# ModelTC/llmc

Hardware: AMD Instinct MI355X
Metric: layers/sec (GPTQ W4A16, Llama-3-8B Linear shapes, 128x2048 calib) (higher is better)
Workload: dtype bf16

## Files before the change

include/llmc_hip.h:

```cpp
#ifndef LLMC_HIP_H_
#define LLMC_HIP_H_

#include <stddef.h>
#include <stdint.h>

#ifdef __cplusplus
extern "C" {
#endif

#define LLMC_HIP_ABI_VERSION 1

#define LLMC_OK 0
#define LLMC_EINVAL (-22)
#define LLMC_ENOTSUP (-95)
#define LLMC_EIO (-5)

#define LLMC_F16 0
#define LLMC_BF16 1
#define LLMC_F32 2
#define LLMC_F64 3
#define LLMC_SCALAR_QPARAM 16
#define LLMC_FRACTIONAL_ZP 32

#define LLMC_OUT_FAKE 0
// ... 108 lines not shown
                                              llmc_stream_t stream);
int llmc_hessian_accum_barrier_timeouts(const void* ws, const int64_t* T_list_host, int n, int64_t K, int64_t ldx,
                                        unsigned* out_host, llmc_stream_t stream);

size_t llmc_hessian_prep_ws_bytes(int64_t K);
int llmc_hessian_prep(float* H, const void* W, int wdt, int64_t R, int64_t K, const int64_t* perm,
                      float percdamp, float* Hout, float* Wout, void* ws, llmc_stream_t stream);

int llmc_gather_cols(const float* in, int64_t R, int64_t K, const int64_t* idx, float* out, llmc_stream_t stream);

size_t llmc_chol_inv_upper_ws_bytes(int64_t K);
int llmc_chol_inv_upper(float* A, int64_t K, void* ws, int32_t* info_dev, llmc_stream_t stream);
int llmc_hessian_prep_rev(float* H, const void* W, int wdt, int64_t R, int64_t K, const int64_t* perm,
                          float percdamp, float* Hout, float* Wout, void* ws, llmc_stream_t stream);
int llmc_chol_inv_upper_rev(float* Arev, float* Uout, int64_t K, void* ws, int32_t* info_dev, llmc_stream_t stream);

size_t llmc_gptq_quantize_ws_bytes(int64_t R, int64_t K);
int llmc_gptq_quantize(float* W, const float* Hinv, int64_t R, int64_t K, int sym, float qmin,
                       float qmax, int64_t group_size, int static_groups, const int32_t* col_group,
                       float* scales, float* zeros, float* Wout, float* losses, int blocksize,
                       void* ws, llmc_stream_t stream);
int llmc_gptq_quantize_cols(float* W, const float* Hinv, int64_t R, int64_t K, int64_t n_quant, int sym, float qmin,
                       float qmax, int64_t group_size, int static_groups, const int32_t* col_group,
                       float* scales, float* zeros, float* Wout, float* losses, int blocksize,
                       void* ws, llmc_stream_t stream);
int llmc_gptq_quantize_fp8_cols(float* W, const float* Hinv, int64_t R, int64_t K, int64_t n_quant, int fmt,
                                int64_t group_size, int static_groups, const int32_t* col_group, float* scales,
                                float* Wout, float* losses, int blocksize, void* ws, llmc_stream_t stream);
size_t llmc_gptq_quantize_mse_ws_bytes(int64_t R, int64_t K);
int llmc_gptq_quantize_mse(float* W, const float* Hinv, int64_t R, int64_t K, int64_t n_quant, int sym, float qmin,
// ... 134 lines not shown
```

llmc_amd/_ffi.py:

```python
import ctypes as C
import os

import torch

_HERE = os.path.dirname(os.path.abspath(__file__))
LIB_PATH = os.path.join(_HERE, 'csrc', 'libllmc_hip.so')

F16, BF16, F32 = 0, 1, 2
F64 = 3
OUT_FAKE, OUT_I32, OUT_I8, OUT_U8 = 0, 1, 2, 3
SCALAR_QPARAM = 16
LINEAR_YBLOCKED = 4
FRACTIONAL_ZP = 32
KV_REQUANT, KV_NEW_FAKE = 1, 2

_DT = {torch.float16: F16, torch.bfloat16: BF16, torch.float32: F32}

_i64, _i32, _f32, _f64, _vp, _sz = C.c_int64, C.c_int, C.c_float, C.c_double, C.c_void_p, C.c_size_t

SIGNATURES = {
    'llmc_hip_abi_version': (_i32, []),
    'llmc_hip_build_id': (C.c_char_p, []),
    'llmc_hip_last_error': (_i32, [C.c_char_p, _sz]),
    'llmc_hip_set_helper_streams': (_i32, [_i32]),
# ... 28 lines not shown
    'llmc_hessian_accum_ptrs_partials': (_i32, [_vp, _vp, _i32, _i32, _i64, _i64, _vp, _vp]),
    'llmc_hessian_accum_ptrs_reduce': (_i32, [_vp, _vp, _i32, _i64, _i64, _f64, _f64, _vp, _vp]),
    'llmc_hessian_accum_barrier_timeouts': (_i32, [_vp, _vp, _i32, _i64, _i64, _vp, _vp]),
    'llmc_hessian_max_problems': (_i32, []),
    'llmc_hessian_accum_multi_ws_bytes': (_sz, [_vp, _i32]),
    'llmc_hessian_accum_multi_partials': (_i32, [_vp, _i32, _i32, _vp, _vp]),
    'llmc_hessian_accum_multi_reduce': (_i32, [_vp, _i32, _vp, _vp]),
    'llmc_hessian_accum_multi_barrier_timeouts': (_i32, [_vp, _i32, _vp, _vp, _vp]),
    'llmc_gather_cols': (_i32, [_vp, _i64, _i64, _vp, _vp, _vp]),
    'llmc_hessian_prep_ws_bytes': (_sz, [_i64]),
    'llmc_hessian_prep': (_i32, [_vp, _vp, _i32, _i64, _i64, _vp, _f32, _vp, _vp, _vp, _vp]),
    'llmc_chol_inv_upper_ws_bytes': (_sz, [_i64]),
    'llmc_chol_inv_upper': (_i32, [_vp, _i64, _vp, _vp, _vp]),
    'llmc_hessian_prep_rev': (_i32, [_vp, _vp, _i32, _i64, _i64, _vp, _f32, _vp, _vp, _vp, _vp]),
    'llmc_chol_inv_upper_rev': (_i32, [_vp, _vp, _i64, _vp, _vp, _vp]),
    'llmc_gptq_quantize_ws_bytes': (_sz, [_i64, _i64]),
    'llmc_gptq_quantize': (_i32, [_vp, _vp, _i64, _i64, _i32, _f32, _f32, _i64, _i32, _vp, _vp, _vp, _vp, _vp,
                                  _i32, _vp, _vp]),
    'llmc_gptq_quantize_cols': (_i32, [_vp, _vp, _i64, _i64, _i64, _i32, _f32, _f32, _i64, _i32, _vp, _vp, _vp, _vp, _vp,
                                       _i32, _vp, _vp]),
    'llmc_gptq_quantize_fp8_cols': (_i32, [_vp, _vp, _i64, _i64, _i64, _i32, _i64, _i32, _vp, _vp, _vp, _vp, _i32, _vp, _vp]),
    'llmc_gptq_quantize_mse_ws_bytes': (_sz, [_i64, _i64]),
    'llmc_gptq_quantize_mse': (_i32, [_vp, _vp, _i64, _i64, _i64, _i32, _f32, _f32, _i64, _i32, _i32, _i32, _f32, _vp, _vp,
                                      _vp, _vp, _i32, _vp, _vp]),
    'llmc_spqr_quantize_ws_bytes': (_sz, [_i64, _i64]),
    'llmc_spqr_quantize': (_i32, [_vp, _vp, _i64, _i64, _f32, _f32, _i64, _f32, _i32, _f32, _f32, _f32, _f32, _vp, _vp,
                                  _vp, _vp, _vp, _i32, _vp, _vp]),
    'llmc_awq_act_mean_ws_bytes': (_sz, [_i64, _i64]),
    'llmc_awq_act_mean': (_i32, [_vp, _i32, _i64, _i64, _vp, _vp, _vp]),
    'llmc_awq_weight_mean_ws_bytes': (_sz, [_i64, _i64]),
# ... 54 lines not shown
    'llmc_kv_sink_update': (_i32, [_i32, _i64, _i64, _i64, _i64, _i64, _i64, _i64, _i64, _i64, _i64, _i64, _vp, _vp, _vp, _vp, _vp,
                                   _vp, _vp, _vp, _i64, _i64, _i64, _vp]),
    'llmc_block_influence_ws_bytes': (_sz, [_i64]),
    'llmc_block_influence': (_i32, [_vp, _vp, _i32, _i64, _i64, _i64, _i64, _i32, _vp, _vp, _vp, _vp]),
    'llmc_test_sgemm': (_i32, [_vp, _vp, _vp, _i64, _i64, _i64, _i32, _i32, _i32, _i32, _i32, _i32, _i32, _i32,
                               _i32, _i32, _vp]),
    'llmc_test_sgemm_phased': (_i32, [_vp, _vp, _vp, _i64, _i64, _i64, _i32, _i32, _i32, _i32, _i32, _vp]),
    'llmc_test_gemm3': (_i32, [_vp, _vp, _vp, _i64, _i64, _i64, _i32, _i32, _i32, _i32, _i32, _i32, _i32, _i32, _vp]),
    'llmc_test_gemm3_planes': (_i32, [_vp, _vp, _vp, _i64, _i64, _i64, _i32, _i32, _i32, _i32, _i32, _vp, _vp]),
    'llmc_test_gemm3s_stamps': (_i32, [_vp]),
    'llmc_test_gptq_rider_plan': (_i32, [_i64, _i64, _i64, _i64, _i32, _vp, _i32]),
    'llmc_test_gptq_pipe_plan': (_i32, [_i64, _i64, _i64, _i64, _i32, _vp, _i32]),
    'llmc_test_chol_plan': (_i32, [_i64, _i32, _i32, _vp, _i32]),
    'llmc_test_gemm_route': (_i32, [_vp, _vp]),
    'llmc_test_linear_route': (_i32, [_vp, _vp]),
}



class HessianProblem(C.Structure):
    _fields_ = [('H', _vp), ('dstate', _vp), ('X_list_host', _vp), ('T_list_host', _vp), ('n', _i32), ('K', _i64),
                ('ldx', _i64), ('n_before', _f64), ('n_after', _f64)]


_lib = None


class LlmcHipError(RuntimeError):
    pass

# ... 172 lines not shown
```

llmc_amd/compression/quantization/gptq_ops.py:

```python
import torch

from llmc_amd import _ffi


def hessian_prep(H, W, perm, percdamp, want_h=True, h_out=None, reverse_h=False):
    _ffi.require_gpu(H, W, perm)
    L = _ffi.lib()
    K = H.shape[0]
    Hout = None
    if want_h:
        Hout = h_out if h_out is not None else torch.empty_like(H)
    Wout = None
    R = 0
    if W is not None:
        R = W.shape[0]
        W = W.contiguous()
        Wout = torch.empty((R, K), dtype=torch.float32, device=W.device)
    ws = _ffi.workspace(L.llmc_hessian_prep_ws_bytes(K), H.device)
    if perm is not None:
        perm = perm.to(torch.int64).contiguous()
    fn = L.llmc_hessian_prep_rev if reverse_h else L.llmc_hessian_prep
    _ffi.check(fn(_ffi.ptr(H), _ffi.ptr(W), _ffi.dt(W) if W is not None else 2, R, K,
                  _ffi.ptr(perm), float(percdamp), _ffi.ptr(Hout), _ffi.ptr(Wout), _ffi.ptr(ws),
                  _ffi.stream()), 'llmc_hessian_prep')
    return Hout, Wout


GATHER_MAX_K = 40960


def gather_cols(src, idx):
    _ffi.require_gpu(src, idx)
    L = _ffi.lib()
    if src.dtype != torch.float32 or src.dim() != 2:
        raise ValueError('gather_cols: src must be fp32 [R, K]')
# ... 129 lines not shown
```

llmc_amd/compression/quantization/gptq_pipeline.py:

```python
from dataclasses import dataclass

import torch

from llmc_amd import _ffi

from . import gptq_ops
from .hessian import HessianAccumulator


@dataclass
class GptqConfig:
    bit: int = 4
    symmetric: bool = False
    group_size: int = 128
    actorder: bool = True
    static_groups: bool = False
    percdamp: float = 0.01
    blocksize: int = 128
    mse: tuple = None

    def __post_init__(self):
        if isinstance(self.bit, str):
            if self.bit not in gptq_ops.FP8_FORMATS:
                raise NotImplementedError(f"GptqConfig bit={self.bit!r}: the FP8 column loop has the e4m3 and e5m2 grids")
# ... 41 lines not shown


def _prep_and_factor(H, W, perm, percdamp, h_work):
    if _ffi.HOST_OPTIONS['k3_fused_prep']:
        Hrev, Wp = gptq_ops.hessian_prep(H, W, perm, percdamp, want_h=True, h_out=h_work, reverse_h=True)
        U, info = gptq_ops.chol_inv_upper_rev(Hrev, check=False, return_info=True)
        return U, Wp, info
    Hp, Wp = gptq_ops.hessian_prep(H, W, perm, percdamp, want_h=True, h_out=h_work)
    U, info = gptq_ops.chol_inv_upper(Hp, check=False, return_info=True)
    return U, Wp, info


def quantize_stacked(W_list, H, cfg, static_qparams=None, h_work=None, want_losses=True, rows=None):
    _ffi.require_gpu(H, *W_list)
    K = H.shape[0]
    Wcat = torch.cat([w.reshape(w.shape[0], -1) for w in W_list], dim=0) if len(W_list) > 1 else W_list[0]
    if rows is not None:
        if static_qparams is not None:
            sc = torch.cat([s.reshape(w.shape[0], -1) for (s, _), w in zip(static_qparams, W_list)], 0)[rows[0]:rows[1]]
            zr = None
            if static_qparams[0][1] is not None:
                zr = torch.cat([z.reshape(w.shape[0], -1) for (_, z), w in zip(static_qparams, W_list)], 0)[rows[0]:rows[1]]
            static_qparams = [(sc, zr)]
        W_list = [Wcat[rows[0]:rows[1]]]
        Wcat = W_list[0]
    rows = [w.shape[0] for w in W_list]
    perm = None
    if cfg.actorder:
        perm = torch.argsort(torch.diagonal(H), descending=True)
    U, Wp, info = _prep_and_factor(H, Wcat, perm, cfg.percdamp, h_work)
    qmin, qmax = cfg.qrange
    static_mode = cfg.static_groups or not cfg.group_size
# ... 72 lines not shown
```

llmc_amd/csrc/abi.hip:

```cpp
#include <mutex>
#include <set>
#include <utility>
#include "common.h"

namespace llmc {
static thread_local char g_last_error[512] = "";
static thread_local int g_helper_streams = 1;
bool helper_streams_enabled() { return g_helper_streams != 0; }
static thread_local int g_cu_reserve = 0;
int cu_reserve() { return g_cu_reserve; }
static thread_local int g_opt[OPT_COUNT] = {};
int opt(int id) { return (id >= 0 && id < OPT_COUNT) ? g_opt[id] : 0; }
static const char* const g_opt_names[OPT_COUNT] = {
    "k3_fp32", "k3_no_gemm6", "k3_no_planes", "k3_split_far", "k4_split_far", "k4_err_rowmajor", "gptq_generic",
    "gemm3_nospec", "gemm3s_min_tiles", "no_shortk", "linear_nosplit", "fp8_exact_div", "side_cu_mask", "k1_batch_off", "k1_fp32_diag", "fp8_no_packed16", "gemm3s_no_dma", "sgemm_no_wide", "gemm3_no_wide", "no_riders", "kv_sink_max_grid",
    "block_influence_max_grid"};

void set_last_error(const char* where, hipError_t e) {
    snprintf(g_last_error, sizeof(g_last_error), "%s: %s (%d)", where, hipGetErrorString(e), (int)e);
}
void set_last_error_msg(const char* msg) { snprintf(g_last_error, sizeof(g_last_error), "%s", msg); }

static std::mutex g_dev_mu;
static int g_cu_count[LLMC_MAX_DEVICES] = {};
static std::set<std::pair<int, const void*>> g_lds_attr_done;

int device_cu_count() {
    int dev = 0;
    if (hipGetDevice(&dev) != hipSuccess || dev < 0 || dev >= LLMC_MAX_DEVICES) return 256;
    std::lock_guard<std::mutex> lk(g_dev_mu);
    if (g_cu_count[dev] == 0) {
// ... 71 lines not shown
```

llmc_amd/csrc/cholesky.hip:

```cpp
#include <stdlib.h>
#include "common.h"
#include "mfma_common.h"
#include "sgemm.h"
#include "pipe_lanes.h"

namespace llmc {

static constexpr int NB = 128;

__global__ __launch_bounds__(256) void k_antitranspose(const float* __restrict__ in, float* __restrict__ out,
                                                       int n, int upper_only) {
    __shared__ float tile[32][33];
    const int tx = threadIdx.x & 31, ty = threadIdx.x >> 5;
    const int r0 = blockIdx.y * 32, c0 = blockIdx.x * 32;
    for (int y = ty; y < 32; y += 8) {
        int r = r0 + y, c = c0 + tx;
        tile[y][tx] = (r < n && c < n) ? in[(int64_t)r * n + c] : 0.0f;
    }
    __syncthreads();
    for (int y = ty; y < 32; y += 8) {
        int c = c0 + y, r = r0 + tx;
        if (r < n && c < n) {
            int orow = n - 1 - c, ocol = n - 1 - r;
            float v = tile[tx][y];
            if (upper_only && ocol < orow) v = 0.0f;
            out[(int64_t)orow * n + ocol] = v;
        }
    }
}

static constexpr int PLD = 132;

__device__ __forceinline__ float rdlane(float v, int l) {
    return __int_as_float(__builtin_amdgcn_readlane(__float_as_int(v), l));
}

__device__ __forceinline__ void wave_potrf32_inv(float* __restrict__ S, float* __restrict__ V,
                                                 float* __restrict__ rowbuf, int lane, int kglobal,
                                                 int* __restrict__ info) {
#pragma clang fp contract(fast)
    (void)rowbuf;
    const int j = lane & 31, h = lane >> 5;
    f32x16 A, E;
// ... 316 lines not shown
template <> __device__ __forceinline__ float4 load4_f32<f16_t>(const f16_t* p) {
    const uint2 u = *reinterpret_cast<const uint2*>(p);
    f16_t h[4];
    __builtin_memcpy(h, &u, 8);
    return make_float4(to_f32<f16_t>(h[0]), to_f32<f16_t>(h[1]), to_f32<f16_t>(h[2]), to_f32<f16_t>(h[3]));
}
template <> __device__ __forceinline__ float4 load4_f32<bf16_t>(const bf16_t* p) {
    const uint2 u = *reinterpret_cast<const uint2*>(p);
    bf16_t h[4];
    __builtin_memcpy(h, &u, 8);
    return make_float4(to_f32<bf16_t>(h[0]), to_f32<bf16_t>(h[1]), to_f32<bf16_t>(h[2]), to_f32<bf16_t>(h[3]));
}

static constexpr int GATHER_ROWS = 8;
static constexpr int GATHER_MAXJ = 7;
template <typename T, int MODE>
__global__ __launch_bounds__(512) void k_gather_lds(const T* __restrict__ in, int K, const int64_t* __restrict__ idx,
                                                   const uint8_t* __restrict__ dead, float percdamp,
                                                   const float* __restrict__ diag_mean, float* __restrict__ out, int64_t R) {
    extern __shared__ __attribute__((aligned(16))) float grow[];
    const float damp = MODE == 2 ? percdamp * (*diag_mean) : 0.0f;
    const int64_t r_begin = (int64_t)blockIdx.x * GATHER_ROWS;
    const int64_t r_end = r_begin + GATHER_ROWS < R ? r_begin + GATHER_ROWS : R;
    for (int c_pass = 0; c_pass < K; c_pass += 4 * 512 * GATHER_MAXJ) {
        int pj[GATHER_MAXJ][4];
        uint32_t deadbits = 0;
#pragma unroll
        for (int j = 0; j < GATHER_MAXJ; ++j) {
            const int c = c_pass + 4 * (int)threadIdx.x + 4 * 512 * j;
#pragma unroll
            for (int t = 0; t < 4; ++t) {
                int v = 0;
                if (c < K) {
                    v = idx ? (int)idx[c + t] : c + t;
                    if (MODE == 1 && dead[v]) deadbits |= 1u << (4 * j + t);
                }
                pj[j][t] = v;
            }
        }
        for (int64_t r = r_begin; r < r_end; ++r) {
            const int64_t sr = (MODE == 2 && idx) ? idx[r] : r;
            const T* src = in + sr * K;
            __syncthreads();
            for (int c = 4 * threadIdx.x; c < K; c += 4 * 512) *reinterpret_cast<float4*>(grow + c) = load4_f32<T>(src + c);
            __syncthreads();
#pragma unroll
            for (int j = 0; j < GATHER_MAXJ; ++j) {
                const int c = c_pass + 4 * (int)threadIdx.x + 4 * 512 * j;
                if (c >= K) break;
                float v[4];
#pragma unroll
                for (int t = 0; t < 4; ++t) {
                    float x = grow[pj[j][t]];
                    if (MODE == 1 && ((deadbits >> (4 * j + t)) & 1u)) x = 0.0f;
                    if (MODE == 2 && r == c + t) x += damp;
                    v[t] = x;
                }
                *reinterpret_cast<float4*>(out + r * K + c) = make_float4(v[0], v[1], v[2], v[3]);
            }
        }
    }
}

static constexpr int GATHER_LDS_MAX = 160 * 1024;

template <typename T, int MODE>
static int gather_lds_launch(const T* in, int64_t R, int64_t K, const int64_t* idx, const uint8_t* dead,
                             float percdamp, const float* diag_mean, float* out, hipStream_t st) {
    if (K * 4 > 65536)
        if (int rc = ensure_dynamic_lds((const void*)k_gather_lds<T, MODE>, GATHER_LDS_MAX)) return rc;
    hipLaunchKernelGGL((k_gather_lds<T, MODE>), dim3((unsigned)ceil_div64(R, GATHER_ROWS)), dim3(512), (size_t)K * 4, st, in,
                       (int)K, idx, dead, percdamp, diag_mean, out, R);
    LLMC_LAUNCH_CHECK();
    return LLMC_OK;
}
static inline bool gather_lds_ok(int64_t K, const void* in, const void* out, int esz) {
    return K % 4 == 0 && K * 4 <= GATHER_LDS_MAX && ((uintptr_t)in % (4 * esz)) == 0 && ((uintptr_t)out & 15) == 0;
}

}

using namespace llmc;

extern "C" int llmc_gather_cols(const float* in, int64_t R, int64_t K, const int64_t* idx, float* out,
                                llmc_stream_t stream) {
    LLMC_REQUIRE(in && idx && out && R > 0 && K > 0, "gather_cols: null/empty argument");
    LLMC_REQUIRE(in != out, "gather_cols: out must not alias in");
// ... 5 lines not shown
}

extern "C" size_t llmc_hessian_prep_ws_bytes(int64_t K) {
    if (K <= 0) return 0;
    return (size_t)(((K + 63) / 64) * 64 + 64) + (size_t)K * 8;
}

namespace llmc {
__global__ __launch_bounds__(256) void k_reverse_perm(const int64_t* __restrict__ perm, int K, int64_t* __restrict__ out) {
    const int i = blockIdx.x * 256 + threadIdx.x;
    if (i < K) out[i] = perm ? perm[K - 1 - i] : (int64_t)(K - 1 - i);
}
}

static int hessian_prep_impl(float* H, const void* W, int wdt, int64_t R, int64_t K, const int64_t* perm, float percdamp,
                             float* Hout, float* Wout, void* ws, llmc_stream_t stream, bool rev) {
    LLMC_REQUIRE(H && ws && K > 0, "hessian_prep: null/empty argument");
    LLMC_REQUIRE((W && Wout && R > 0) || (!W && !Wout), "hessian_prep: W and Wout go together");
    LLMC_REQUIRE(dtype_ok(wdt), "hessian_prep: bad dtype");
    LLMC_REQUIRE(Hout != H, "hessian_prep: Hout must not alias H");
    LLMC_REQUIRE(K < (1ll << 31) && R < 65536ll * 32768ll, "hessian_prep: shape too large");
    hipStream_t st = (hipStream_t)stream;
    float* diag_mean = (float*)ws;
    uint8_t* dead = (uint8_t*)ws + 64;
    hipLaunchKernelGGL(k_diag_fix, dim3(1), dim3(1024), 0, st, H, (int)K, dead, diag_mean);
    LLMC_LAUNCH_CHECK();
    int gx = (int)ceil_div64(K, 256 * 4);
    if (Hout) {
        const int64_t* hperm = perm;
        if (rev) {
            int64_t* pr = (int64_t*)((char*)ws + (((K + 63) / 64) * 64 + 64));
            hipLaunchKernelGGL(k_reverse_perm, dim3((unsigned)ceil_div64(K, 256)), dim3(256), 0, st, perm, (int)K, pr);
            LLMC_LAUNCH_CHECK();
            hperm = pr;
        }
        if (gather_lds_ok(K, H, Hout, 4)) {
            int rc = gather_lds_launch<float, 2>(H, K, K, hperm, nullptr, percdamp, diag_mean, Hout, st);
            if (rc) return rc;
        } else {
            hipLaunchKernelGGL(k_gather_h, dim3(gx, (unsigned)K), dim3(256), 0, st, (const float*)H, (int)K, hperm,
                               percdamp, (const float*)diag_mean, Hout);
            LLMC_LAUNCH_CHECK();
        }
    }
    if (W && gather_lds_ok(K, W, Wout, wdt == LLMC_F32 ? 4 : 2)) {
        int rc;
        if (wdt == LLMC_F16) rc = gather_lds_launch<f16_t, 1>((const f16_t*)W, R, K, perm, dead, 0.0f, nullptr, Wout, st);
        else if (wdt == LLMC_BF16)
            rc = gather_lds_launch<bf16_t, 1>((const bf16_t*)W, R, K, perm, dead, 0.0f, nullptr, Wout, st);
        else rc = gather_lds_launch<float, 1>((const float*)W, R, K, perm, dead, 0.0f, nullptr, Wout, st);
        return rc;
    }
    for (int64_t r0 = 0; W && r0 < R; r0 += 32768) {
        int64_t rows = R - r0 < 32768 ? R - r0 : 32768;
        dim3 grid(gx, (unsigned)rows);
        if (wdt == LLMC_F16)
            hipLaunchKernelGGL((k_gather_w<f16_t>), grid, dim3(256), 0, st, (const f16_t*)W + r0 * K, rows, (int)K,
                               perm, (const uint8_t*)dead, Wout + r0 * K);
        else if (wdt == LLMC_BF16)
// ... 3 lines not shown
            hipLaunchKernelGGL((k_gather_w<float>), grid, dim3(256), 0, st, (const float*)W + r0 * K, rows, (int)K,
                               perm, (const uint8_t*)dead, Wout + r0 * K);
        LLMC_LAUNCH_CHECK();
    }
    return LLMC_OK;
}

extern "C" int llmc_hessian_prep(float* H, const void* W, int wdt, int64_t R, int64_t K, const int64_t* perm,
                                 float percdamp, float* Hout, float* Wout, void* ws, llmc_stream_t stream) {
    return hessian_prep_impl(H, W, wdt, R, K, perm, percdamp, Hout, Wout, ws, stream, false);
}

extern "C" int llmc_hessian_prep_rev(float* H, const void* W, int wdt, int64_t R, int64_t K, const int64_t* perm,
                                     float percdamp, float* Hout, float* Wout, void* ws, llmc_stream_t stream) {
    return hessian_prep_impl(H, W, wdt, R, K, perm, percdamp, Hout, Wout, ws, stream, true);
}

static inline size_t align256(size_t x) { return (x + 255) & ~(size_t)255; }

static constexpr int64_t GEMM6_MIN_H = 4096;
static size_t gemm6_bytes(int64_t K) {
    size_t mx = 0;
    for (int64_t h = NB; h < K; h *= 2)
        if (h >= GEMM6_MIN_H) {
            const size_t b = gemm6_ws_bytes((int)h, (int)h, (int)h);
            if (b > mx) mx = b;
        }
    return align256(mx);
}

// ... 102 lines not shown
            const int64_t off = f - (x ? o.Xbuf : (const float*)o.G6buf);
            return Rect{x ? 2 : 3, 0, 1, (int32_t)off, (int32_t)(off + (rows - 1) * ld + cols)};
        }
        const bool v = f >= o.Vbuf && f < o.Xbuf, w = f >= o.Wk && f < o.Wk + (size_t)o.K * o.K;
        const int64_t n = v ? NB : o.K, off = f - (v ? o.Vbuf : w ? o.Wk : other);
        return Rect{ld != n ? -2 : v ? 1 : w ? 0 : 4, (int32_t)(off / n), (int32_t)(off / n + rows), (int32_t)(off % n), (int32_t)(off % n + cols)};
    }
    int add(int kind, int form, Lane lane, Rect w, Rect a = Rect{-1}, Rect b = Rect{-1}, Rect w2 = Rect{-1}) const {
        int32_t v[CP_W] = {kind, form};
        memcpy(v + 2, &w, sizeof w), memcpy(v + 7, &a, sizeof a), memcpy(v + 12, &b, sizeof b), memcpy(v + 17, &w2, sizeof w2);
        rec->row(v, ln.lane_of(ln.s[lane]));
        return LLMC_OK;
    }
    int transpose(const float* in, float* out, int upper_only) const {
        if (rec) return add(CP_TRANSPOSE, F_KERNEL, CHAIN, rect(out, o.K, o.K, o.K), rect(in, o.K, o.K, o.K));
        hipLaunchKernelGGL(k_antitranspose, dim3((o.K + 31) / 32, (o.K + 31) / 32), dim3(256), 0, ln.s[CHAIN], in, out, o.K, upper_only);
        return launched();
    }
    int potrf(int c0, int nb) const {
        float* Vb = o.V(c0);
        if (rec) return add(CP_POTRF, F_KERNEL, CHAIN, rect(o.at(c0, c0), o.K, nb, nb), rect(o.at(c0, c0), o.K, nb, nb), Rect{-1}, rect(Vb, NB, nb, NB));
        hipLaunchKernelGGL(k_potrf_inv, dim3(1), dim3(256), POTRF_LDS, ln.s[CHAIN], o.Wk, (int64_t)o.K, c0, nb, Vb, info);
        return launched();
    }
    int product(int kind, const SgemmArgs& g, int form, bool TA, Lane lane) const {
        if (g.M <= 0 || g.N <= 0) return LLMC_OK;
        const hipStream_t st = ln.s[lane];
        if (!rec) return form == F_SGEMM ? sgemm_launch(g, TA, false, st) : gemm3_launch(g, TA, st);
        auto hull = [&](const float* p, int64_t ld, int64_t s, int r, int c, int rl, int cl) {
            const Rect a = rect(p, ld, r, c), b = rect(p + (g.batch - 1) * s, ld, rl, cl);
            return Rect{a.buf, a.r0, b.r1, a.c0, b.c1};
// ... 99 lines not shown
}

extern "C" int llmc_chol_inv_upper_rev(float* Arev, float* Uout, int64_t K64, void* ws, int32_t* info_dev, llmc_stream_t stream) {
    LLMC_REQUIRE(Uout && Uout != Arev && ((uintptr_t)Uout & 15) == 0, "chol_inv_upper_rev: Uout must be a separate 16-B aligned buffer");
    return chol_inv_upper_impl(Arev, Uout, K64, ws, info_dev, stream);
}

extern "C" int llmc_test_chol_plan(int64_t K, int rev, int with_lanes, int32_t* out, int cap) {
    LLMC_REQUIRE(out && cap >= 0, "chol plan: null output");
    PlanRec rec{out, cap, 0, CP_W, with_lanes != 0, CP_BLANK};
    float* const base = (float*)(uintptr_t)((uint64_t)1 << 40);
    const size_t span = (size_t)1 << 36;
    const int rc = chol_inv_upper_impl(base, rev ? base + span : nullptr, K, base + 2 * span, (int32_t*)(base + 3 * span), nullptr, &rec);
    return rc ? rc : rec.n;
}
```

llmc_amd/csrc/common.h:

```cpp
#pragma once
#include <hip/hip_runtime.h>
#include <stdint.h>
#include <string.h>
#include <stdio.h>
#include <stdlib.h>
#include <type_traits>

#include "../../include/llmc_hip.h"

namespace llmc {

void set_last_error(const char* where, hipError_t e);
void set_last_error_msg(const char* msg);

#define LLMC_HIP_CHECK(expr)                                   \
    do {                                                       \
        hipError_t _e = (expr);                                \
        if (_e != hipSuccess) {                                \
            ::llmc::set_last_error(#expr, _e);                 \
            return LLMC_EIO;                                   \
        }                                                      \
    } while (0)

#define LLMC_LAUNCH_CHECK()                                    \
// ... 30 lines not shown
    OPT_GEMM3_NOSPEC,
    OPT_GEMM3S_MIN_TILES,
    OPT_NO_SHORTK,
    OPT_LINEAR_NOSPLIT,
    OPT_FP8_EXACT_DIV,
    OPT_SIDE_CU_MASK,
    OPT_K1_BATCH_OFF,
    OPT_K1_FP32_DIAG,
    OPT_FP8_NO_PACKED16,
    OPT_GEMM3S_NO_DMA,
    OPT_SGEMM_NO_WIDE,
    OPT_GEMM3_NO_WIDE,
    OPT_NO_RIDERS,
    OPT_KV_SINK_MAX_GRID,
    OPT_BLOCK_INFLUENCE_MAX_GRID,
    OPT_COUNT
};
int opt(int id);
#ifdef LLMC_LAB
static inline const char* lab_env(const char* k) { return getenv(k); }
#endif

static inline int dtype_size(int dt) { return dt == LLMC_F32 ? 4 : 2; }
static inline bool dtype_ok(int dt) { return dt == LLMC_F16 || dt == LLMC_BF16 || dt == LLMC_F32; }

struct f16_t { uint16_t u; };
struct bf16_t { uint16_t u; };

template <typename T> struct dt_of;
template <> struct dt_of<f16_t> { static constexpr int value = LLMC_F16; };
// ... 114 lines not shown
```

llmc_amd/csrc/hessian_syrk.hip:

```cpp
#include <stdlib.h>
#include "common.h"
#include "mfma_common.h"

namespace llmc {

static constexpr int TM = 256;
static constexpr int TILE_FLOATS = TM * TM;
static constexpr int GROUP_TOK = 128;
static constexpr int SYRK_MAX_SAMPLES = 512;
static constexpr int SYRK_MAX_CHUNKS = 32;
static constexpr int SYRK_UNIT_SAMPLES = 64;
static constexpr int FOLD_GROUPS = 16;
static constexpr int SYRK_MAX_PROBS = 4;

struct TileIdx {
    int bi, bj;
    bool valid;
};

__host__ __device__ inline int tiles_padded(int nb) {
    int sb = (nb + 3) / 4;
    return 8 * sb * sb + 2 * sb;
}
__host__ __device__ inline TileIdx decode_tile(int ti, int nb) {
// ... 446 lines not shown
        int i = i0 + r;
        if (i < K) {
            float h = a.beta * sum[r];
            if (a.alpha != 0.0f) h += a.alpha * H[(int64_t)i * K + j];
            o[r] = h;
            if (!(fa.exact && i == j)) H[(int64_t)i * K + j] = h;
        }
    }
    if (t.bi != t.bj || (dtile && wm == 1 && wn < 2)) {
#pragma unroll
        for (int r = 0; r < 4; ++r)
            if (i0 + r < K) H[(int64_t)j * K + i0 + r] = o[r];
    }
}

struct DiagProb {
    const double* dpart;
    double* dstate;
    float* H;
    int K, nbK, S, pad_;
    double alpha, beta;
};
struct DiagArgs {
    DiagProb pr[SYRK_MAX_PROBS];
};

__global__ __launch_bounds__(256) void k_diag_apply(const DiagArgs da) {
    const DiagProb& a = da.pr[blockIdx.y];
    const int j = blockIdx.x * 256 + threadIdx.x;
    if (j >= a.K) return;
// ... 197 lines not shown
        const llmc_hessian_problem_t& h = probs_host[q];
        LLMC_REQUIRE(h.H && h.n_after > 0, "hessian_accum_reduce: bad argument");
        const SyrkProb& p = a.pr[q];
        f.pr[q].part = p.part; f.pr[q].H = h.H; f.pr[q].K = p.K; f.pr[q].nb = p.nb; f.pr[q].ntiles_p = p.ntiles_p; f.pr[q].S = p.S;
        f.pr[q].alpha = (float)(h.n_before / h.n_after);
        f.pr[q].beta = (float)(2.0 / h.n_after);
        d.pr[q].dpart = p.dpart; d.pr[q].dstate = h.dstate; d.pr[q].H = h.H; d.pr[q].K = p.K; d.pr[q].nbK = p.nb * TM; d.pr[q].S = p.S;
        d.pr[q].pad_ = 0;
        d.pr[q].alpha = h.n_before / h.n_after;
        d.pr[q].beta = 2.0 / h.n_after;
        if (p.ntiles_p > max_tiles) max_tiles = p.ntiles_p;
        if (p.K > max_k) max_k = p.K;
    }
    f.exact = exact ? 1 : 0;
    hipStream_t st = (hipStream_t)stream;
    hipLaunchKernelGGL(k_syrk_fixup, dim3(TILE_FLOATS / 4 / 256, max_tiles, P), dim3(256), 0, st, f);
    LLMC_LAUNCH_CHECK();
    if (exact) {
        hipLaunchKernelGGL(k_diag_apply, dim3((unsigned)ceil_div64(max_k, 256), P), dim3(256), 0, st, d);
        LLMC_LAUNCH_CHECK();
    }
    return LLMC_OK;
}

extern "C" int llmc_hessian_accum_multi_barrier_timeouts(const llmc_hessian_problem_t* probs_host, int P, const void* ws,
                                                         unsigned* out_host, llmc_stream_t stream) {
    LLMC_REQUIRE(ws && out_host, "hessian_accum_barrier_timeouts: null argument");
    SyrkArgs a;
    int rc = syrk_plan_multi(probs_host, P, (void*)ws, &a, nullptr);
    if (rc) return rc;
    unsigned w[2 * SYRK_MAX_PROBS] = {};
    LLMC_HIP_CHECK(hipMemcpyAsync(w, a.sync, sizeof(w), hipMemcpyDeviceToHost, (hipStream_t)stream));
    LLMC_HIP_CHECK(hipStreamSynchronize((hipStream_t)stream));
    unsigned t = 0;
    for (int q = 0; q < SYRK_MAX_PROBS; ++q) t += w[2 * q + 1];
    *out_host = t;
// ... 62 lines not shown
```

Before: 79.86.

## Gather stacked weights directly, vectorize antitranspose, and transpose SYRK fixup mirror writes via LDS

Adds a stacked hessian_prep path that gathers rows straight from up to eight separate weight tensors, so q/k/v or gate/up no longer need a torch.cat copy first. Adds a float4 antitranspose kernel that also skips loading dead lower tiles when only the upper triangle is wanted. Replaces the SYRK fixup mirror store, which wrote strided scalars, with an LDS-staged transpose that writes coalesced float4 rows. The old fixup kernel stays reachable behind an option flag. Together these cut memory traffic in Hessian preparation, at the cost of more kernel variants and extra alignment preconditions.

```diff
diff --git a/include/llmc_hip.h b/include/llmc_hip.h
--- a/include/llmc_hip.h
+++ b/include/llmc_hip.h
@@ -146,6 +146,9 @@
 int llmc_hessian_prep_rev(float* H, const void* W, int wdt, int64_t R, int64_t K, const int64_t* perm,
                           float percdamp, float* Hout, float* Wout, void* ws, llmc_stream_t stream);
 int llmc_chol_inv_upper_rev(float* Arev, float* Uout, int64_t K, void* ws, int32_t* info_dev, llmc_stream_t stream);
+int llmc_hessian_prep_stack(float* H, const void* const* W_list_host, const int64_t* R_list_host, int n, int wdt, int64_t K,
+                            const int64_t* perm, float percdamp, float* Hout, float* Wout, int reverse_h, void* ws,
+                            llmc_stream_t stream);
 
 size_t llmc_gptq_quantize_ws_bytes(int64_t R, int64_t K);
 int llmc_gptq_quantize(float* W, const float* Hinv, int64_t R, int64_t K, int sym, float qmin,
diff --git a/llmc_amd/_ffi.py b/llmc_amd/_ffi.py
--- a/llmc_amd/_ffi.py
+++ b/llmc_amd/_ffi.py
@@ -66,6 +66,7 @@
     'llmc_chol_inv_upper': (_i32, [_vp, _i64, _vp, _vp, _vp]),
     'llmc_hessian_prep_rev': (_i32, [_vp, _vp, _i32, _i64, _i64, _vp, _f32, _vp, _vp, _vp, _vp]),
     'llmc_chol_inv_upper_rev': (_i32, [_vp, _vp, _i64, _vp, _vp, _vp]),
+    'llmc_hessian_prep_stack': (_i32, [_vp, _vp, _vp, _i32, _i32, _i64, _vp, _f32, _vp, _vp, _i32, _vp, _vp]),
     'llmc_gptq_quantize_ws_bytes': (_sz, [_i64, _i64]),
     'llmc_gptq_quantize': (_i32, [_vp, _vp, _i64, _i64, _i32, _f32, _f32, _i64, _i32, _vp, _vp, _vp, _vp, _vp,
                                   _i32, _vp, _vp]),
@@ -150,6 +151,9 @@
     'llmc_test_chol_plan': (_i32, [_i64, _i32, _i32, _vp, _i32]),
     'llmc_test_gemm_route': (_i32, [_vp, _vp]),
     'llmc_test_linear_route': (_i32, [_vp, _vp]),
+    'llmc_test_hessian_chunks': (_i32, [_vp, _i32, _vp]),
+    'llmc_test_gather_lds': (_i32, [_vp, _i32, _i32, _i64, _i64, _vp, _vp, _f32, _vp, _vp, _vp]),
+    'llmc_test_antitranspose':(_i32, [_vp, _vp, _i64, _i32, _vp]),
 }
 
 
diff --git a/llmc_amd/compression/quantization/gptq_ops.py b/llmc_amd/compression/quantization/gptq_ops.py
--- a/llmc_amd/compression/quantization/gptq_ops.py
+++ b/llmc_amd/compression/quantization/gptq_ops.py
@@ -1,15 +1,40 @@
+import ctypes as C
+
 import torch
 
 from llmc_amd import _ffi
 
+STACK_MAX_SOURCES = 8
+ENOTSUP = -95
+
 
 def hessian_prep(H, W, perm, percdamp, want_h=True, h_out=None, reverse_h=False):
-    _ffi.require_gpu(H, W, perm)
+    if isinstance(W, (list, tuple)):
+        W = [w.reshape(w.shape[0], -1) for w in W]
+        W = W[0] if len(W) == 1 else W
+    Ws = W if isinstance(W, list) else None
+    _ffi.require_gpu(H, perm, *(Ws or [W]))
     L = _ffi.lib()
     K = H.shape[0]
     Hout = None
     if want_h:
         Hout = h_out if h_out is not None else torch.empty_like(H)
+    if perm is not None:
+        perm = perm.to(torch.int64).contiguous()
+    if Ws is not None:
+        Ws = [w.contiguous() for w in Ws]
+        if len(Ws) <= STACK_MAX_SOURCES and len({w.dtype for w in Ws}) == 1:
+            Wout = torch.empty((sum(w.shape[0] for w in Ws), K), dtype=torch.float32, device=H.device)
+            ws = _ffi.workspace(L.llmc_hessian_prep_ws_bytes(K), H.device)
+            n = len(Ws)
+            rc = L.llmc_hessian_prep_stack(_ffi.ptr(H), (C.c_void_p * n)(*[w.data_ptr() for w in Ws]),
+                                           (C.c_int64 * n)(*[w.shape[0] for w in Ws]), n, _ffi.dt(Ws[0]), K, _ffi.ptr(perm),
+                                           float(percdamp), _ffi.ptr(Hout), _ffi.ptr(Wout), int(bool(reverse_h)), _ffi.ptr(ws),
+                                           _ffi.stream())
+            if rc != ENOTSUP:
+                _ffi.check(rc, 'llmc_hessian_prep_stack')
+                return Hout, Wout
+        W = torch.cat(Ws, dim=0)
     Wout = None
     R = 0
     if W is not None:
@@ -17,8 +42,6 @@
         W = W.contiguous()
         Wout = torch.empty((R, K), dtype=torch.float32, device=W.device)
     ws = _ffi.workspace(L.llmc_hessian_prep_ws_bytes(K), H.device)
-    if perm is not None:
-        perm = perm.to(torch.int64).contiguous()
     fn = L.llmc_hessian_prep_rev if reverse_h else L.llmc_hessian_prep
     _ffi.check(fn(_ffi.ptr(H), _ffi.ptr(W), _ffi.dt(W) if W is not None else 2, R, K,
                   _ffi.ptr(perm), float(percdamp), _ffi.ptr(Hout), _ffi.ptr(Wout), _ffi.ptr(ws),
diff --git a/llmc_amd/compression/quantization/gptq_pipeline.py b/llmc_amd/compression/quantization/gptq_pipeline.py
--- a/llmc_amd/compression/quantization/gptq_pipeline.py
+++ b/llmc_amd/compression/quantization/gptq_pipeline.py
@@ -79,8 +79,9 @@
 def quantize_stacked(W_list, H, cfg, static_qparams=None, h_work=None, want_losses=True, rows=None):
     _ffi.require_gpu(H, *W_list)
     K = H.shape[0]
-    Wcat = torch.cat([w.reshape(w.shape[0], -1) for w in W_list], dim=0) if len(W_list) > 1 else W_list[0]
+    Wcat = list(W_list)
     if rows is not None:
+        Wcat = torch.cat([w.reshape(w.shape[0], -1) for w in W_list], dim=0) if len(W_list) > 1 else W_list[0]
         if static_qparams is not None:
             sc = torch.cat([s.reshape(w.shape[0], -1) for (s, _), w in zip(static_qparams, W_list)], 0)[rows[0]:rows[1]]
             zr = None
diff --git a/llmc_amd/csrc/abi.hip b/llmc_amd/csrc/abi.hip
--- a/llmc_amd/csrc/abi.hip
+++ b/llmc_amd/csrc/abi.hip
@@ -14,7 +14,7 @@
 static const char* const g_opt_names[OPT_COUNT] = {
     "k3_fp32", "k3_no_gemm6", "k3_no_planes", "k3_split_far", "k4_split_far", "k4_err_rowmajor", "gptq_generic",
     "gemm3_nospec", "gemm3s_min_tiles", "no_shortk", "linear_nosplit", "fp8_exact_div", "side_cu_mask", "k1_batch_off", "k1_fp32_diag", "fp8_no_packed16", "gemm3s_no_dma", "sgemm_no_wide", "gemm3_no_wide", "no_riders", "kv_sink_max_grid",
-    "block_influence_max_grid"};
+    "block_influence_max_grid", "k1_fixup_direct"};
 
 void set_last_error(const char* where, hipError_t e) {
     snprintf(g_last_error, sizeof(g_last_error), "%s: %s (%d)", where, hipGetErrorString(e), (int)e);
diff --git a/llmc_amd/csrc/cholesky.hip b/llmc_amd/csrc/cholesky.hip
--- a/llmc_amd/csrc/cholesky.hip
+++ b/llmc_amd/csrc/cholesky.hip
@@ -3,6 +3,7 @@
 #include "mfma_common.h"
 #include "sgemm.h"
 #include "pipe_lanes.h"
+#include "gather_stack.h"
 
 namespace llmc {
 
@@ -13,9 +14,10 @@
     __shared__ float tile[32][33];
     const int tx = threadIdx.x & 31, ty = threadIdx.x >> 5;
     const int r0 = blockIdx.y * 32, c0 = blockIdx.x * 32;
+    const bool dead_tile = upper_only && r0 > c0 + 31;
     for (int y = ty; y < 32; y += 8) {
         int r = r0 + y, c = c0 + tx;
-        tile[y][tx] = (r < n && c < n) ? in[(int64_t)r * n + c] : 0.0f;
+        tile[y][tx] = (!dead_tile && r < n && c < n) ? in[(int64_t)r * n + c] : 0.0f;
     }
     __syncthreads();
     for (int y = ty; y < 32; y += 8) {
@@ -27,6 +29,37 @@
             out[(int64_t)orow * n + ocol] = v;
         }
     }
+}
+
+__global__ __launch_bounds__(256) void k_antitranspose4(const float* __restrict__ in, float* __restrict__ out, int n, int upper_only) {
+    __shared__ float tile[32][33];
+    const int x4 = 4 * (threadIdx.x & 7), y = threadIdx.x >> 3;
+    const int r0 = blockIdx.y * 32, c0 = blockIdx.x * 32;
+    const bool dead_tile = upper_only && r0 > c0 + 31;
+    {
+        const int r = r0 + y, c = c0 + x4;
+        float4 v = make_float4(0.f, 0.f, 0.f, 0.f);
+        if (!dead_tile && r < n && c < n) v = *reinterpret_cast<const float4*>(in + (int64_t)r * n + c);
+        tile[y][x4] = v.x, tile[y][x4 + 1] = v.y, tile[y][x4 + 2] = v.z, tile[y][x4 + 3] = v.w;
+    }
+    __syncthreads();
+    const int c = c0 + y, r = r0 + x4;
+    if (r < n && c < n) {
+        const int orow = n - 1 - c, ocol = n - 4 - r;
+        float v[4];
+#pragma unroll
+        for (int t = 0; t < 4; ++t) {
+            v[t] = tile[x4 + 3 - t][y];
+            if (upper_only && ocol + t < orow) v[t] = 0.0f;
+        }
+        *reinterpret_cast<float4*>(out + (int64_t)orow * n + ocol) = make_float4(v[0], v[1], v[2], v[3]);
+    }
+}
+
+static inline void antitranspose_launch(const float* in, float* out, int n, int upper_only, hipStream_t st) {
+    const bool wide = n % 4 == 0 && (((uintptr_t)in | (uintptr_t)out) & 15) == 0;
+    hipLaunchKernelGGL(wide ? k_antitranspose4 : k_antitranspose, dim3((n + 31) / 32, (n + 31) / 32), dim3(256), 0, st, in, out, n,
+                       upper_only);
 }
 
 static constexpr int PLD = 132;
@@ -373,10 +406,10 @@
 
 static constexpr int GATHER_ROWS = 8;
 static constexpr int GATHER_MAXJ = 7;
-template <typename T, int MODE>
-__global__ __launch_bounds__(512) void k_gather_lds(const T* __restrict__ in, int K, const int64_t* __restrict__ idx,
-                                                   const uint8_t* __restrict__ dead, float percdamp,
-                                                   const float* __restrict__ diag_mean, float* __restrict__ out, int64_t R) {
+template <typename T, int MODE, typename RowSrc>
+__device__ __forceinline__ void gather_lds_rows(RowSrc row_src, int K, const int64_t* __restrict__ idx,
+                                                const uint8_t* __restrict__ dead, float percdamp,
+                                                const float* __restrict__ diag_mean, float* __restrict__ out, int64_t R) {
     extern __shared__ __attribute__((aligned(16))) float grow[];
     const float damp = MODE == 2 ? percdamp * (*diag_mean) : 0.0f;
     const int64_t r_begin = (int64_t)blockIdx.x * GATHER_ROWS;
@@ -398,8 +431,7 @@
             }
         }
         for (int64_t r = r_begin; r < r_end; ++r) {
-            const int64_t sr = (MODE == 2 && idx) ? idx[r] : r;
-            const T* src = in + sr * K;
+            const T* src = row_src(r);
             __syncthreads();
             for (int c = 4 * threadIdx.x; c < K; c += 4 * 512) *reinterpret_cast<float4*>(grow + c) = load4_f32<T>(src + c);
             __syncthreads();
@@ -421,15 +453,42 @@
     }
 }
 
+template <typename T, int MODE>
+__global__ __launch_bounds__(512) void k_gather_lds(const T* __restrict__ in, int K, const int64_t* __restrict__ idx,
+                                                   const uint8_t* __restrict__ dead, float percdamp,
+                                                   const float* __restrict__ diag_mean, float* __restrict__ out, int64_t R) {
+    gather_lds_rows<T, MODE>([=](int64_t r) { return in + ((MODE == 2 && idx) ? idx[r] : r) * K; }, K, idx, dead, percdamp,
+                             diag_mean, out, R);
+}
+
+template <typename T>
+__global__ __launch_bounds__(512) void k_gather_lds_stack(const GatherStack st, int K, const int64_t* __restrict__ idx,
+                                                         const uint8_t* __restrict__ dead, float* __restrict__ out, int64_t R) {
+    gather_lds_rows<T, 1>([&](int64_t r) { return (const T*)gather_stack_row(st, r, (int64_t)K * sizeof(T)); }, K, idx, dead, 0.0f,
+                          nullptr, out, R);
+}
+
 static constexpr int GATHER_LDS_MAX = 160 * 1024;
 
 template <typename T, int MODE>
 static int gather_lds_launch(const T* in, int64_t R, int64_t K, const int64_t* idx, const uint8_t* dead,
                              float percdamp, const float* diag_mean, float* out, hipStream_t st) {
-    if (K * 4 > 65536)
+    const size_t lds = (size_t)K * 4;
+    if (lds > 65536)
         if (int rc = ensure_dynamic_lds((const void*)k_gather_lds<T, MODE>, GATHER_LDS_MAX)) return rc;
-    hipLaunchKernelGGL((k_gather_lds<T, MODE>), dim3((unsigned)ceil_div64(R, GATHER_ROWS)), dim3(512), (size_t)K * 4, st, in,
+    hipLaunchKernelGGL((k_gather_lds<T, MODE>), dim3((unsigned)ceil_div64(R, GATHER_ROWS)), dim3(512), lds, st, in,
                        (int)K, idx, dead, percdamp, diag_mean, out, R);
+    LLMC_LAUNCH_CHECK();
+    return LLMC_OK;
+}
+template <typename T>
+static int gather_stack_launch(const GatherStack& t, int64_t R, int64_t K, const int64_t* idx, const uint8_t* dead, float* out,
+                               hipStream_t st) {
+    const size_t lds = (size_t)K * 4;
+    if (lds > 65536)
+        if (int rc = ensure_dynamic_lds((const void*)k_gather_lds_stack<T>, GATHER_LDS_MAX)) return rc;
+    hipLaunchKernelGGL((k_gather_lds_stack<T>), dim3((unsigned)ceil_div64(R, GATHER_ROWS)), dim3(512), lds, st, t, (int)K,
+                       idx, dead, out, R);
     LLMC_LAUNCH_CHECK();
     return LLMC_OK;
 }
@@ -465,7 +524,8 @@
 }
 
 static int hessian_prep_impl(float* H, const void* W, int wdt, int64_t R, int64_t K, const int64_t* perm, float percdamp,
-                             float* Hout, float* Wout, void* ws, llmc_stream_t stream, bool rev) {
+                             float* Hout, float* Wout, void* ws, llmc_stream_t stream, bool rev, const GatherStack* stack = nullptr) {
+    if (stack) W = stack->p[0];
     LLMC_REQUIRE(H && ws && K > 0, "hessian_prep: null/empty argument");
     LLMC_REQUIRE((W && Wout && R > 0) || (!W && !Wout), "hessian_prep: W and Wout go together");
     LLMC_REQUIRE(dtype_ok(wdt), "hessian_prep: bad dtype");
@@ -494,6 +554,12 @@
             LLMC_LAUNCH_CHECK();
         }
     }
+    if (stack) {
+        const uint8_t* dd = dead;
+        if (wdt == LLMC_F16) return gather_stack_launch<f16_t>(*stack, R, K, perm, dd, Wout, st);
+        if (wdt == LLMC_BF16) return gather_stack_launch<bf16_t>(*stack, R, K, perm, dd, Wout, st);
+        return gather_stack_launch<float>(*stack, R, K, perm, dd, Wout, st);
+    }
     if (W && gather_lds_ok(K, W, Wout, wdt == LLMC_F32 ? 4 : 2)) {
         int rc;
         if (wdt == LLMC_F16) rc = gather_lds_launch<f16_t, 1>((const f16_t*)W, R, K, perm, dead, 0.0f, nullptr, Wout, st);
@@ -527,6 +593,22 @@
 extern "C" int llmc_hessian_prep_rev(float* H, const void* W, int wdt, int64_t R, int64_t K, const int64_t* perm,
                                      float percdamp, float* Hout, float* Wout, void* ws, llmc_stream_t stream) {
     return hessian_prep_impl(H, W, wdt, R, K, perm, percdamp, Hout, Wout, ws, stream, true);
+}
+
+extern "C" int llmc_hessian_prep_stack(float* H, const void* const* W_list_host, const int64_t* R_list_host, int n, int wdt,
+                                       int64_t K, const int64_t* perm, float percdamp, float* Hout, float* Wout, int reverse_h,
+                                       void* ws, llmc_stream_t stream) {
+    LLMC_REQUIRE(H && ws && K > 0 && W_list_host && R_list_host && Wout && n >= 1, "hessian_prep_stack: null/empty argument");
+    LLMC_REQUIRE(dtype_ok(wdt), "hessian_prep_stack: bad dtype");
+    GatherStack t;
+    const int64_t R = gather_stack_build(W_list_host, R_list_host, n, 65536ll * 32768ll - 1, &t);
+    bool ok = R > 0;
+    for (int s = 0; ok && s < n; ++s) ok = gather_lds_ok(K, W_list_host[s], Wout, wdt == LLMC_F32 ? 4 : 2);
+    if (!ok) {
+        set_last_error_msg("hessian_prep_stack: 1 .. 8 sources, each with K % 4 == 0, K <= 40960 and rows aligned to four elements");
+        return LLMC_ENOTSUP;
+    }
+    return hessian_prep_impl(H, nullptr, wdt, R, K, perm, percdamp, Hout, Wout, ws, stream, reverse_h != 0, &t);
 }
 
 static inline size_t align256(size_t x) { return (x + 255) & ~(size_t)255; }
@@ -659,7 +741,7 @@
     }
     int transpose(const float* in, float* out, int upper_only) const {
         if (rec) return add(CP_TRANSPOSE, F_KERNEL, CHAIN, rect(out, o.K, o.K, o.K), rect(in, o.K, o.K, o.K));
-        hipLaunchKernelGGL(k_antitranspose, dim3((o.K + 31) / 32, (o.K + 31) / 32), dim3(256), 0, ln.s[CHAIN], in, out, o.K, upper_only);
+        antitranspose_launch(in, out, o.K, upper_only, ln.s[CHAIN]);
         return launched();
     }
     int potrf(int c0, int nb) const {
@@ -789,3 +871,24 @@
     const int rc = chol_inv_upper_impl(base, rev ? base + span : nullptr, K, base + 2 * span, (int32_t*)(base + 3 * span), nullptr, &rec);
     return rc ? rc : rec.n;
 }
+
+extern "C" int llmc_test_gather_lds(const void* in, int dt, int mode, int64_t R, int64_t K, const int64_t* idx, const uint8_t* dead,
+                                    float percdamp, const float* diag_mean, float* out, llmc_stream_t stream) {
+    LLMC_REQUIRE(in && out && R > 0 && K > 0 && K < (1ll << 31) && dtype_ok(dt), "test_gather_lds: bad argument");
+    LLMC_REQUIRE(mode == 0 || (mode == 1 && dead) || (mode == 2 && diag_mean), "test_gather_lds: mode 1 needs dead, mode 2 diag_mean");
+    LLMC_REQUIRE(dt == LLMC_F32 || mode == 1, "test_gather_lds: 16-bit sources are mode 1's");
+    if (!gather_lds_ok(K, in, out, dt == LLMC_F32 ? 4 : 2)) return LLMC_ENOTSUP;
+    hipStream_t st = (hipStream_t)stream;
+    if (dt == LLMC_F16) return gather_lds_launch<f16_t, 1>((const f16_t*)in, R, K, idx, dead, 0.0f, nullptr, out, st);
+    if (dt == LLMC_BF16) return gather_lds_launch<bf16_t, 1>((const bf16_t*)in, R, K, idx, dead, 0.0f, nullptr, out, st);
+    if (mode == 1) return gather_lds_launch<float, 1>((const float*)in, R, K, idx, dead, 0.0f, nullptr, out, st);
+    if (mode == 2) return gather_lds_launch<float, 2>((const float*)in, R, K, idx, nullptr, percdamp, diag_mean, out, st);
+    return gather_lds_launch<float, 0>((const float*)in, R, K, idx, nullptr, 0.0f, nullptr, out, st);
+}
+
+extern "C" int llmc_test_antitranspose(const float* in, float* out, int64_t n, int upper_only, llmc_stream_t stream) {
+    LLMC_REQUIRE(in && out && in != out && n > 0 && n < (1ll << 31), "test_antitranspose: bad argument");
+    antitranspose_launch(in, out, (int)n, upper_only, (hipStream_t)stream);
+    LLMC_LAUNCH_CHECK();
+    return LLMC_OK;
+}
diff --git a/llmc_amd/csrc/common.h b/llmc_amd/csrc/common.h
--- a/llmc_amd/csrc/common.h
+++ b/llmc_amd/csrc/common.h
@@ -68,6 +68,7 @@
     OPT_NO_RIDERS,
     OPT_KV_SINK_MAX_GRID,
     OPT_BLOCK_INFLUENCE_MAX_GRID,
+    OPT_K1_FIXUP_DIRECT,
     OPT_COUNT
 };
 int opt(int id);
diff --git a/llmc_amd/csrc/gather_stack.h b/llmc_amd/csrc/gather_stack.h
--- /dev/null
+++ b/llmc_amd/csrc/gather_stack.h
@@ -0,0 +1,41 @@
+#pragma once
+#include <stdint.h>
+
+namespace llmc {
+
+static constexpr int GATHER_MAX_SRC = 8;
+struct GatherStack {
+    const void* p[GATHER_MAX_SRC];
+    int64_t r0[GATHER_MAX_SRC];
+};
+
+static inline int64_t gather_stack_build(const void* const* W, const int64_t* R, int n, int64_t max_rows, GatherStack* t) {
+    if (!W || !R || !t || n < 1 || n > GATHER_MAX_SRC) return -1;
+    int64_t total = 0;
+    for (int s = 0; s < GATHER_MAX_SRC; ++s) {
+        if (s >= n) {
+            t->p[s] = nullptr;
+            t->r0[s] = INT64_MAX;
+            continue;
+        }
+        if (!W[s] || R[s] <= 0 || R[s] > max_rows - total) return -1;
+        t->p[s] = W[s];
+        t->r0[s] = total;
+        total += R[s];
+    }
+    return total;
+}
+
+#ifdef __HIPCC__
+__host__ __device__
+#endif
+static inline const void* gather_stack_row(const GatherStack& t, int64_t r, int64_t row_bytes) {
+    const void* base = t.p[0];
+    int64_t rb = 0;
+#pragma unroll
+    for (int s = 1; s < GATHER_MAX_SRC; ++s)
+        if (r >= t.r0[s]) base = t.p[s], rb = t.r0[s];
+    return (const char*)base + (r - rb) * row_bytes;
+}
+
+}
diff --git a/llmc_amd/csrc/hessian_syrk.hip b/llmc_amd/csrc/hessian_syrk.hip
--- a/llmc_amd/csrc/hessian_syrk.hip
+++ b/llmc_amd/csrc/hessian_syrk.hip
@@ -484,6 +484,82 @@
     }
 }
 
+static constexpr int FIX_LD = 36;
+__global__ __launch_bounds__(256) void k_syrk_fixup_t(const FixupArgs fa) {
+    __shared__ __attribute__((aligned(16))) float mt[32 * FIX_LD];
+    const FixupProb& a = fa.pr[blockIdx.z];
+    const int ti = blockIdx.y;
+    if (ti >= a.ntiles_p) return;
+    const TileIdx t = decode_tile(ti, a.nb);
+    if (!t.valid) return;
+    const int idx = blockIdx.x * 256 + threadIdx.x;
+    const int lane = idx & 63;
+    const int q = (idx >> 6) & 3;
+    const int n = (idx >> 8) & 1;
+    const int m = (idx >> 9) & 3;
+    const int wv = idx >> 11;
+    const int wm = wv >> 2, wn = wv & 3;
+    const bool dtile = fa.exact && t.bi == t.bj;
+    if (dtile && wm == 0 && wn >= 2) return;
+    f32x4 sum = {0.f, 0.f, 0.f, 0.f};
+    const int64_t sstride = (int64_t)a.ntiles_p * TILE_FLOATS;
+    const float* src = a.part + (int64_t)ti * TILE_FLOATS + (int64_t)idx * 4;
+    int s = 0;
+    for (; s + 4 <= a.S; s += 4) {
+        const f32x4 v0 = *reinterpret_cast<const f32x4*>(src);
+        const f32x4 v1 = *reinterpret_cast<const f32x4*>(src + sstride);
+        const f32x4 v2 = *reinterpret_cast<const f32x4*>(src + 2 * sstride);
+        const f32x4 v3 = *reinterpret_cast<const f32x4*>(src + 3 * sstride);
+        sum += v0;
+        sum += v1;
+        sum += v2;
+        sum += v3;
+        src += 4 * sstride;
+    }
+    {
+        const int rem = a.S - s;
+        f32x4 v0 = {0.f, 0.f, 0.f, 0.f}, v1 = v0, v2 = v0;
+        if (rem > 0) v0 = *reinterpret_cast<const f32x4*>(src);
+        if (rem > 1) v1 = *reinterpret_cast<const f32x4*>(src + sstride);
+        if (rem > 2) v2 = *reinterpret_cast<const f32x4*>(src + 2 * sstride);
+        if (rem > 0) sum += v0;
+        if (rem > 1) sum += v1;
+        if (rem > 2) sum += v2;
+    }
+    const int K = a.K;
+    float* H = a.H;
+    const int rb = t.bi * TM + wm * 128 + m * 32, jb = t.bj * TM + wn * 64 + n * 32;
+    const int ro = 8 * q + 4 * (lane >> 5), jo = lane & 31;
+    const int i0 = rb + ro, j = jb + jo;
+    f32x4 o = {0.f, 0.f, 0.f, 0.f};
+    if (j < K) {
+#pragma unroll
+        for (int r = 0; r < 4; ++r) {
+            int i = i0 + r;
+            if (i < K) {
+                float h = a.beta * sum[r];
+                if (a.alpha != 0.0f) h += a.alpha * H[(int64_t)i * K + j];
+                o[r] = h;
+                if (!(fa.exact && i == j)) H[(int64_t)i * K + j] = h;
+            }
+        }
+    }
+    if (!(t.bi != t.bj || (dtile && wm == 1 && wn < 2))) return;
+    *reinterpret_cast<f32x4*>(mt + jo * FIX_LD + ro) = o;
+    __syncthreads();
+    const int mr = jb + ((int)threadIdx.x >> 3), mc = rb + 4 * ((int)threadIdx.x & 7);
+    if (mr >= K || mc >= K) return;
+    const f32x4 v = *reinterpret_cast<const f32x4*>(mt + ((int)threadIdx.x >> 3) * FIX_LD + 4 * ((int)threadIdx.x & 7));
+    float* dst = H + (int64_t)mr * K + mc;
+    if ((K & 3) == 0 && ((uintptr_t)H & 15) == 0) {
+        *reinterpret_cast<f32x4*>(dst) = v;
+    } else {
+#pragma unroll
+        for (int r = 0; r < 4; ++r)
+            if (mc + r < K) dst[r] = v[r];
+    }
+}
+
 struct DiagProb {
     const double* dpart;
     double* dstate;
@@ -711,12 +787,23 @@
     }
     f.exact = exact ? 1 : 0;
     hipStream_t st = (hipStream_t)stream;
-    hipLaunchKernelGGL(k_syrk_fixup, dim3(TILE_FLOATS / 4 / 256, max_tiles, P), dim3(256), 0, st, f);
+    const dim3 fgrid(TILE_FLOATS / 4 / 256, max_tiles, P);
+    if (opt(OPT_K1_FIXUP_DIRECT)) hipLaunchKernelGGL(k_syrk_fixup, fgrid, dim3(256), 0, st, f);
+    else hipLaunchKernelGGL(k_syrk_fixup_t, fgrid, dim3(256), 0, st, f);
     LLMC_LAUNCH_CHECK();
     if (exact) {
         hipLaunchKernelGGL(k_diag_apply, dim3((unsigned)ceil_div64(max_k, 256), P), dim3(256), 0, st, d);
         LLMC_LAUNCH_CHECK();
     }
+    return LLMC_OK;
+}
+
+extern "C" int llmc_test_hessian_chunks(const llmc_hessian_problem_t* probs_host, int P, int* S_out_host) {
+    LLMC_REQUIRE(S_out_host, "test_hessian_chunks: null argument");
+    SyrkArgs a;
+    int rc = syrk_plan_multi(probs_host, P, nullptr, &a, nullptr);
+    if (rc) return rc;
+    for (int q = 0; q < P; ++q) S_out_host[q] = a.pr[q].S;
     return LLMC_OK;
 }
 
```

New measurement: 80.26 (median of 6 runs). About the same (+0.5%).
